# venkovic/julia-phd-krylov-spdes

Hardware: AMD Instinct MI355X
Metric: Schur-PCG iterations/sec (NN-preconditioned, assembled local Schurs), 1M DoF (higher is better)
Workload: dtype f64; 1 GPU; configs[2]: N=1000 structured P1 mesh, 996004 free DoF, 8 subdomains (4x2 boxes), lognormal a=exp(g) seed 481456, n_Γ=3989; pcg(S, b_schur, 0, ΠSnn), eps=1e-07; subdomains_per_gpu=8, parallelism=single GPU, it=15

## Files before the change

### julia-phd-krylov-spdes_amd/csrc/kernels.hpp

```cpp
#pragma once
#include <hip/hip_runtime.h>

#include "exchange_dev.hpp"
#include "spmv_blocks.hpp"

namespace mi {

constexpr int NT = 256;
constexpr int MAX_PARTS = 512;

struct SolverState {
  double rTr, rTz;
  double rTr_prev, rTz_prev;
  double d, alpha, beta;
  double tol, bnorm, eps;
  long long it, maxit, res_cap;
  long long it_nxt;
  int done;
  int overflow;
  int x0_zero;
};

struct PinnedFlags {
  long long it;
  int done;
  int overflow;
  int respec;
  int x0z;
  long long t_entry, t_exit;
  unsigned long long seq;
};
struct SolveArgs {
  const double *b_in, *x_in;
  double *x_out, *res_stage;
  double eps;
  long long maxit, res_cap, ncap;
  unsigned long long seq;
};

__device__ __forceinline__ double wave_sum(double v) {
#pragma unroll
  for (int off = 32; off > 0; off >>= 1) v += __shfl_down(v, off, 64);
  return v;
}
template <int NTH>
__device__ __forceinline__ double block_sum_t(double v, double *sm) {
  constexpr int NW = NTH / 64;
  v = wave_sum(v);
  const int lane = threadIdx.x & 63, w = threadIdx.x >> 6;
  if (lane == 0) sm[w] = v;
  __syncthreads();
  double t = lane < NW ? sm[lane] : 0.0;
#pragma unroll
  for (int off = NW / 2; off > 0; off >>= 1) t += __shfl_down(t, off, 64);
  t = __shfl(t, 0, 64);
  __syncthreads();
  return t;
}
__device__ __forceinline__ double block_sum(double v, double *sm) { return block_sum_t<NT>(v, sm); }
template <int NTH>
__device__ __forceinline__ void block_sum2_t(double &a, double &b, double *sm) {
// ... 941 lines not shown
  double *res_norm;
  const int *tgt;
  const int *peer;
  const int *jrank;
  int W;
  const unsigned long long *in_epoch;
  long long in_stride;
  const XchgPeers *xp;
  XchgState *xst;
  long long out_stride;
  unsigned int n_arrive;
  const XchgPeers *xpw;
  int x_inwait;
  int nvec;
  long long n_gamma;
  const double *AW;
  double *part_mu;
  const double *wm_loc;
  const SolveArgs *exit_args;
  PinnedFlags *exit_flags;
  long long *dbg;
  int dbg_wg;
};
#define MI_FSTAMP(i) \
  do { if (f.dbg && (int)blockIdx.x == f.dbg_wg && threadIdx.x == 0) f.dbg[dbg_row * 8 + (i)] = wall_clock64(); } while (0)
__device__ __forceinline__ double slot_sum(const double *slots, int g, int W) {
  double s = 0.0;
  if (W == 4) {
    const double4 q = *reinterpret_cast<const double4 *>(slots + 4ll * g);
    s += q.x; s += q.y; s += q.z; s += q.w;
  } else if (W == 2) {
    const double2 q = *reinterpret_cast<const double2 *>(slots + 2ll * g);
    s += q.x; s += q.y;
  } else {
    for (int j = 0; j < W; ++j) s += slots[(long long)g * W + j];
  }
  return s;
}

template <int RPW, int PHASE, int FOLD_CPT, int WAVES, bool XCHG, typename MT = double>
__global__ __launch_bounds__(64 * WAVES) void k_gemv_pcg(DenseMeta m, PcgFold f) {
  constexpr int NTH = 64 * WAVES, NR = WAVES * RPW;
  SolverState *st = f.st;
  const bool x_push = XCHG && f.xp != nullptr, x_inwait = XCHG && f.x_inwait != 0;
  const GemvTile t = m.tiles[blockIdx.x];
  const int done0 = st->done;
  const long long it0 = st->it, it_nxt0 = st->it_nxt, maxit = st->maxit, cap = st->res_cap;
  const double tol = st->tol, rTz0 = st->rTz, old = st->rTz_prev;
  const unsigned long long xo = XCHG && f.xst ? (x_inwait ? f.xst->xep[PHASE] : f.xst->epoch) : 0ull;
  const unsigned long long xe = x_inwait ? xo : (f.in_epoch ? *f.in_epoch : 0ull);
  asm volatile("" ::"s"(t.mat_off), "s"(t.n), "s"(t.ld), "s"(t.loc_off), "s"(t.row0), "s"(t.active), "s"(t.nrows), "s"(it0),
               "s"(it_nxt0), "s"(maxit), "s"(cap), "s"(tol), "s"(rTz0), "s"(old), "s"(done0), "s"(xe), "s"(xo));
  if (done0) return;
  GemvRows<RPW, MT> rows;
  if (x_inwait && f.in_stride) {
    if (t.active) rows.begin(m, t);
    if (threadIdx.x < 64) xchg_wait(f.xst, *f.xpw, xo);
    __syncthreads();
    if (__hip_atomic_load(&f.xst->err, __ATOMIC_RELAXED, __HIP_MEMORY_SCOPE_AGENT)) return;
  }
  const bool streaming = x_inwait && f.in_stride;
  const long long xoff = (long long)(xe & 1ull) * f.in_stride;
  const double *con_in = f.con_in + xoff, *part_in0 = f.part_in0 + xoff, *part_in1 = PHASE == 0 ? f.part_in1 + xoff : nullptr;
  __shared__ __attribute__((aligned(16))) double xs[GEMV_PANEL];
  __shared__ double sm[2 * (NTH / 64)];
  __shared__ double rowv[NR], rowc0[NR], rowc1[NR];
  __shared__ double rowy[NR];
  __shared__ int rowg[NR];
  const int off = t.loc_off, W = f.W, n = t.n;
  const bool lead = blockIdx.x == 0 && threadIdx.x == 0;
  if (threadIdx.x < NR) { rowc0[threadIdx.x] = 0.0; rowv[threadIdx.x] = 0.0; rowy[threadIdx.x] = 0.0; rowg[threadIdx.x] = 0; }
#if !MI355_OPERAND_FIRST
  if (t.active && !streaming) rows.begin(m, t);
#endif

  const bool first1 = PHASE == 1 && it_nxt0 == 0;
  const int dbg_row = (int)((PHASE == 1 ? 2 * it_nxt0 : 2 * it0 + 1) & 63);
  MI_FSTAMP(0);
  double pa = 0.0, pb = 0.0;
  for (int i0 = threadIdx.x; i0 < f.n_in; i0 += 8 * NTH) {
    double ta[8], tb[8];
#pragma unroll
    for (int k = 0; k < 8; ++k) {
      const int i = i0 + k * NTH;
      ta[k] = i < f.n_in ? part_in0[i] : 0.0;
      tb[k] = PHASE == 0 && i < f.n_in ? part_in1[i] : 0.0;
    }
#pragma unroll
    for (int k = 0; k < 8; ++k) { pa += ta[k]; if (PHASE == 0) pb += tb[k]; }
  }
  double cv[FOLD_CPT], cs[FOLD_CPT], cc[FOLD_CPT];
#pragma unroll
  for (int q = 0; q < FOLD_CPT; ++q) {
    const int j = q * NTH + threadIdx.x;
    cv[q] = cs[q] = 0.0; cc[q] = PHASE == 1 ? 1.0 : 0.0;
    if (j < n) {
      const int loc = off + j;
      cs[q] = slot_sum(con_in, loc, W);
      if (PHASE == 1) { cv[q] = first1 ? f.r_gamma[m.gidx[loc]] : f.r_cur[loc]; cc[q] = m.cnt[loc]; }
      else { cv[q] = f.p_cur[loc]; if (f.nvec > 0) cc[q] = f.wm_loc[loc]; }
    }
  }
  int o_q = -1, o_g = 0;
  bool o_own = false;
  double o_a = 0.0, o_x = 0.0;
  int o_peer[4] = {-1, -1, -1, -1};
#pragma unroll
  for (int q = 0; q < FOLD_CPT; ++q) {
    const int j = q * NTH + threadIdx.x, ri = j - t.row0;
    if (j < n && ri >= 0 && ri < t.nrows) {
      const int loc = off + j;
      o_q = q;
      o_own = f.jrank[loc] == 0;
      if (PHASE == 1) { o_a = first1 ? 0.0 : f.p_nxt[loc]; o_g = m.gidx[loc]; }
      else o_a = f.r_nxt[loc];
#pragma unroll
      for (int k = 0; k < 4; ++k) if (k < W) o_peer[k] = f.peer[loc * W + k];
    }
  }
  if (PHASE == 1 && o_q >= 0 && o_own) o_x = f.x[o_g];
  int e_tgt[RPW][4];
  double e_cnt[RPW];
#pragma unroll
  for (int k = 0; k < RPW; ++k) {
    const int r = t.row0 + (int)(threadIdx.x >> 6) * RPW + k;
    e_cnt[k] = 1.0;
#pragma unroll
    for (int q = 0; q < 4; ++q) e_tgt[k][q] = -1;
    if ((threadIdx.x & 63) == 0 && r < n) {
      const int loc = off + r;
      if (PHASE == 1) e_cnt[k] = m.cnt[loc];
#pragma unroll
      for (int q = 0; q < 4; ++q) if (q < W) e_tgt[k][q] = f.tgt[loc * W + q];
    }
  }

  int x_tgt = -1;
  if (x_push && t.active && threadIdx.x < 4 * NR) {
    const int r = t.row0 + (int)(threadIdx.x >> 2), k = threadIdx.x & 3;
    if (r < n && k < W) x_tgt = f.tgt[(off + r) * W + k];
  }
#if MI355_OPERAND_FIRST
  if (t.active && !streaming) rows.begin(m, t);
#endif
  MI_FSTAMP(1);
  double coef;
  if (PHASE == 1) {
    const bool first = first1;
    block_sum2_t<NTH>(pa, pb, sm);
    const double d = pa;
    coef = first ? 0.0 : rTz0 / d;
    if (lead) {
      st->d = d; st->alpha = coef;
      st->rTz_prev = first ? 1.0 : rTz0;
      st->it = it_nxt0;
      if (x_inwait) { f.xst->xep[0] = xo + (x_push ? 1 : 0); f.xst->epoch = xo; }
    }
  } else {
    const long long it_new = it0 + 1;
    block_sum2_t<NTH>(pa, pb, sm);
    const double rr = pa, rz = pb;
    const double res = sqrt(rr);
    const bool stop = !((it_new < maxit) && (res > tol));
    coef = 1. / old;
    coef *= rz;
    if (lead) {
      st->rTr = rr; st->rTz = rz; st->beta = coef;
      st->it_nxt = it_new;
      if (it_new <= cap) f.res_norm[it_new - 1] = res; else st->overflow = 1;
      if (stop || it_new > cap) st->done = 1;
      if (x_inwait) { f.xst->xep[1] = xo + (x_push && !(stop || it_new > cap) ? 1 : 0); f.xst->epoch = xo; }
    }
    if (stop || it_new > cap) {
      if (f.exit_args && blockIdx.x == 0) {
        const SolveArgs q = *f.exit_args;
        for (long long i = threadIdx.x; i < f.n_gamma; i += NTH) q.x_out[i] = f.x[i];
        if (q.res_stage) {
          const long long mres = it_new < q.ncap ? it_new : q.ncap;
          for (long long i = threadIdx.x; i < mres; i += NTH) q.res_stage[i] = i == it_new - 1 ? res : f.res_norm[i];
        }
        __threadfence_system();
        __syncthreads();
        if (threadIdx.x == 0) {
          PinnedFlags *fl = f.exit_flags;
          fl->it = it_new; fl->done = 1; fl->overflow = it_new > cap; fl->respec = 0; fl->x0z = st->x0_zero;
          fl->t_exit = wall_clock64();
          __threadfence_system();
          __hip_atomic_store(&fl->seq, q.seq, __ATOMIC_RELEASE, __HIP_MEMORY_SCOPE_SYSTEM);
        }
      }
      return;
    }
  }

  MI_FSTAMP(2);
#pragma unroll
  for (int q = 0; q < FOLD_CPT; ++q) {
    const int j = q * NTH + threadIdx.x;
    if (j < t.ld) {
      double v = 0.0, vs = 0.0;
      if (j < n) {
        v = PHASE == 1 ? (first1 ? cv[q] : cv[q] + (-coef) * cs[q])
                       : coef * cv[q] + cs[q];
        if (PHASE == 0 && f.nvec > 0) v = v - cc[q];
        vs = PHASE == 1 ? v / cc[q] : v;
      }
      xs[j] = vs;
      if (q == o_q) {
        const int ri = j - t.row0;
// ... 87 lines not shown
        const XchgPeers &P = *f.xp;
        const char *own = P.arena[P.rank];
        for (int q = 0; q < P.n; ++q) {
          const long long d = P.arena[q] - own;
          xchg_store(reinterpret_cast<double *>(reinterpret_cast<char *>(f.part_out0) + d) + xpo + ps, PHASE == 1 ? b : a);
          if (PHASE == 1) xchg_store(reinterpret_cast<double *>(reinterpret_cast<char *>(f.part_out1) + d) + xpo + ps, a);
        }
      }
    }
  }
  if (x_push) {
    asm volatile("s_waitcnt vmcnt(0)" ::: "memory");
    __syncthreads();
    if (threadIdx.x == 0) {
      const unsigned int prev = __hip_atomic_fetch_add(&f.xst->arrived, 1u, __ATOMIC_RELAXED, __HIP_MEMORY_SCOPE_AGENT);
      if (prev == f.n_arrive - 1) {
        __hip_atomic_store(&f.xst->arrived, 0u, __ATOMIC_RELAXED, __HIP_MEMORY_SCOPE_AGENT);
        const XchgPeers &P = *f.xp;
        for (int q = 0; q < P.n; ++q) __hip_atomic_store(xchg_flag(P, q, P.rank), xo + 1, __ATOMIC_RELAXED, __HIP_MEMORY_SCOPE_SYSTEM);
      }
    }
  }
  MI_FSTAMP(6);
}

__global__ __launch_bounds__(NT) void k_assemble(int n, const int *__restrict__ aptr, const int *__restrict__ apos,
                                                 const double *__restrict__ yloc, double *__restrict__ y,
                                                 const int *done) {
  if (done && *done) return;
  for (int i = blockIdx.x * NT + threadIdx.x; i < n; i += gridDim.x * NT) {
    double s = 0.0;
    for (int k = aptr[i]; k < aptr[i + 1]; ++k) s += yloc[apos[k]];
    y[i] = s;
  }
}
__global__ __launch_bounds__(NT) void k_assemble_slots(int n, int width, const double *__restrict__ yslots,
                                                       double *__restrict__ y, const int *done) {
  if (done && *done) return;
  for (int i = blockIdx.x * NT + threadIdx.x; i < n; i += gridDim.x * NT) {
    double s = 0.0;
    for (int j = 0; j < width; ++j) s += yslots[(long long)i * width + j];
    y[i] = s;
  }
}
__global__ __launch_bounds__(NT) void k_gather(int nloc, const int *__restrict__ gidx, const double *__restrict__ x,
                                               double *__restrict__ xcat) {
// ... 151 lines not shown
  }
  if (blockIdx.x == 0 && threadIdx.x == 0) {
    st->rTr = rr; st->rTz = rz; st->beta = beta;
    const long long it = st->it + 1;
    st->it = it;
    const double res = sqrt(rr);
    const bool over = it > st->res_cap;
    if (!over) res_norm[it - 1] = res; else st->overflow = 1;
    st->done = over || !((it < st->maxit) && (res > st->tol));
  }
}
__global__ __launch_bounds__(NT) void k_solve_begin(int n, const double *__restrict__ b_in, const double *__restrict__ x_in,
                                                    double *__restrict__ b, double *__restrict__ x, SolverState *st, double eps,
                                                    long long maxit, long long res_cap) {
  int nz = 0;
  for (int i = blockIdx.x * NT + threadIdx.x; i < n; i += gridDim.x * NT) {
    const double xi = x_in[i];
    b[i] = b_in[i]; x[i] = xi;
    nz |= xi != 0.0;
  }
  if (__syncthreads_or(nz) && threadIdx.x == 0) st->x0_zero = 0;
  if (blockIdx.x == 0 && threadIdx.x == 0) { st->eps = eps; st->maxit = maxit; st->res_cap = res_cap; st->done = 0; }
}
__device__ __forceinline__ unsigned long long sys_load_u64(const void *p) {
  return __hip_atomic_load((const unsigned long long *)p, __ATOMIC_RELAXED, __HIP_MEMORY_SCOPE_SYSTEM);
}
__global__ __launch_bounds__(NT) void k_solve_begin_g(int n, const SolveArgs *pin, double *__restrict__ b, double *__restrict__ x,
                                                      SolverState *st, SolveArgs *dev, PinnedFlags *flags) {
  __shared__ unsigned long long a[sizeof(SolveArgs) / 8];
  if (blockIdx.x == 0 && threadIdx.x == 0) flags->t_entry = wall_clock64();
  static_assert(sizeof(SolveArgs) % 8 == 0 && sizeof(SolveArgs) / 8 <= 64, "SolveArgs is a block of 8-byte fields");
  if (threadIdx.x < sizeof(SolveArgs) / 8) a[threadIdx.x] = sys_load_u64((const unsigned long long *)pin + threadIdx.x);
  __syncthreads();
  const SolveArgs &q = *reinterpret_cast<const SolveArgs *>(a);
  const double *b_in = q.b_in, *x_in = q.x_in;
  int nz = 0;
  for (int i = blockIdx.x * NT + threadIdx.x; i < n; i += gridDim.x * NT) {
    const double xi = x_in[i];
    b[i] = b_in[i]; x[i] = xi;
    nz |= xi != 0.0;
  }
  if (__syncthreads_or(nz) && threadIdx.x == 0) st->x0_zero = 0;
  if (blockIdx.x == 0) {
    if (threadIdx.x < sizeof(SolveArgs) / 8) ((unsigned long long *)dev)[threadIdx.x] = a[threadIdx.x];
    if (threadIdx.x == 0) { st->eps = q.eps; st->maxit = q.maxit; st->res_cap = q.res_cap; st->done = 0; }
  }
}
__global__ __launch_bounds__(NT) void k_solve_end_g(int n, SolverState *st, const SolveArgs *dev, int fold, const double *__restrict__ x,
                                                    const double *__restrict__ res_norm, PinnedFlags *flags, int *x0_zero,
                                                    unsigned *end_count) {
  __shared__ int last;
  const long long it = fold ? st->it_nxt : st->it;
  const SolveArgs q = *dev;
  if (sys_load_u64(&flags->seq) == q.seq) {
    if (blockIdx.x == 0 && threadIdx.x == 0) *x0_zero = 1;
    return;
  }
  for (int i = blockIdx.x * NT + threadIdx.x; i < n; i += gridDim.x * NT) q.x_out[i] = x[i];
  if (q.res_stage) {
    const long long m = it < q.ncap ? it : q.ncap;
    for (long long i = blockIdx.x * (long long)NT + threadIdx.x; i < m; i += (long long)gridDim.x * NT) q.res_stage[i] = res_norm[i];
  }
  __threadfence_system();
  __syncthreads();
  if (threadIdx.x == 0) last = atomicAdd(end_count, 1u) == gridDim.x - 1;
  __syncthreads();
  if (last && threadIdx.x == 0) {
    *end_count = 0;
    flags->it = it; flags->done = st->done; flags->overflow = st->overflow; flags->respec = 0; flags->x0z = *x0_zero;
    flags->t_exit = wall_clock64();
    *x0_zero = 1;
    __threadfence_system();
    __hip_atomic_store(&flags->seq, q.seq, __ATOMIC_RELEASE, __HIP_MEMORY_SCOPE_SYSTEM);
  }
}
__global__ __launch_bounds__(NT) void k_solve_end(int n, const SolverState *st, int fold, const double *__restrict__ x,
                                                  double *__restrict__ x_out, const double *__restrict__ res_norm,
// ... 376 lines not shown
__global__ __launch_bounds__(NTF) void k_entry_zero(int n, const SolveArgs *pin, double *__restrict__ b, double *__restrict__ x,
                                                    double *__restrict__ r, SolverState *st, SolveArgs *dev, PinnedFlags *flags) {
  __shared__ unsigned long long a[sizeof(SolveArgs) / 8];
  __shared__ double sm[NTF / 64 + 1];
  if (threadIdx.x == 0) flags->t_entry = wall_clock64();
  if (threadIdx.x < sizeof(SolveArgs) / 8) a[threadIdx.x] = sys_load_u64((const unsigned long long *)pin + threadIdx.x);
  __syncthreads();
  const SolveArgs &q = *reinterpret_cast<const SolveArgs *>(a);
  const double *b_in = q.b_in, *x_in = q.x_in;
  double bv[EPT], xv[EPT];
  int nz = 0;
#pragma unroll
  for (int k = 0; k < EPT; ++k) {
    const int e = k * NTF + threadIdx.x;
    bv[k] = 0.0; xv[k] = 0.0;
    if (e < n) { bv[k] = b_in[e]; xv[k] = x_in[e]; nz |= xv[k] != 0.0; }
  }
  nz = __syncthreads_or(nz);
  if (threadIdx.x < sizeof(SolveArgs) / 8) ((unsigned long long *)dev)[threadIdx.x] = a[threadIdx.x];
  if (nz) {
    if (threadIdx.x == 0) {
      st->done = 1; st->x0_zero = 0;
      flags->it = 0; flags->done = 0; flags->overflow = 0; flags->respec = 1; flags->x0z = 0;
      __threadfence_system();
      __hip_atomic_store(&flags->seq, q.seq, __ATOMIC_RELEASE, __HIP_MEMORY_SCOPE_SYSTEM);
    }
    return;
  }
  double srr = 0.0, sbb = 0.0;
#pragma unroll
  for (int k = 0; k < EPT; ++k) {
    const int e = k * NTF + threadIdx.x;
    if (e < n) {
      const double bi = bv[k];
      const double ri = bi - 0.0;
      b[e] = bi; x[e] = xv[k]; r[e] = ri;
      srr += ri * ri;
      sbb += bi * bi;
    }
  }
  srr = block_sum_f(srr, sm);
  sbb = block_sum_f(sbb, sm);
  if (threadIdx.x == 0) {
    st->eps = q.eps; st->maxit = q.maxit; st->res_cap = q.res_cap; st->x0_zero = 1;
    st->rTr = srr; st->bnorm = sqrt(sbb);
    st->tol = q.eps * st->bnorm;
// ... 140 lines not shown
```

### julia-phd-krylov-spdes_amd/csrc/operators.hpp

```cpp
#pragma once
#include <algorithm>
#include <atomic>
#include <cfloat>
#include <cmath>
#include <cstdlib>
#include <functional>
#include <numeric>

#include "common.hpp"
#include "kernels.hpp"
#include "assembly.hpp"
#include "exchange.hpp"

namespace mi {

inline int vec_grid(int64_t n) {
  int64_t g = (n + (int64_t)NT * 4 - 1) / ((int64_t)NT * 4);
  return (int)std::max<int64_t>(1, std::min<int64_t>(g, MAX_PARTS));
}
inline int env_int(const char *name, int dflt) {
  const char *s = std::getenv(name);
  return s && *s ? std::atoi(s) : dflt;
}
inline int to_i32(int64_t v, int64_t lo, int64_t hi, const char *what) {
// ... 461 lines not shown
    hipLaunchKernelGGL(k_assemble_slots, dim3(vec_grid(n)), dim3(NT), 0, ctx->stream, (int)n, maps.slot_width,
                       reduce_over_ranks ? yslots_all.p : yslots.p, y, done);
    MI_HIP(hipGetLastError());
  }
  DenseBlockOp *as_dense() override { return this; }
  void set_blocks(const double *src);
  static constexpr int KV = 4;
  DevBuf<double> yslots_multi;
  void apply_multi(const double *X, int64_t ldx, int k, double *Y, int64_t ldy) override {
    if (reduce_over_ranks || !ntiles || f32() || env_int("MI355_NO_MULTI", 0)) { Operator::apply_multi(X, ldx, k, Y, ldy); return; }
    const long long stride = (long long)n * maps.slot_width + 4;
    if (yslots_multi.n < (size_t)(stride * KV)) { yslots_multi.alloc((size_t)(stride * KV)); yslots_multi.zero(ctx->stream); }
    for (int v0 = 0; v0 < k; v0 += KV) {
      const int kv = std::min(KV, k - v0);
      const double *Xv = X + (size_t)v0 * ldx;
#define MI_GM(S) hipLaunchKernelGGL((k_gemv_multi<2, KV, S, 16>), dim3(ntiles), dim3(1024), 0, ctx->stream, meta, Xv, (long long)ldx, kv, yslots_multi.p, stride)
      if (scale) MI_GM(true); else MI_GM(false);
#undef MI_GM
      hipLaunchKernelGGL(k_assemble_slots_multi, dim3(vec_grid(n), kv), dim3(NT), 0, ctx->stream, (int)n, maps.slot_width,
                         yslots_multi.p, stride, Y + (size_t)v0 * ldy, (long long)ldy);
    }
    MI_HIP(hipGetLastError());
  }
  void gemv_pcg(int phase, const PcgFold &f) {
    if (!ntiles) return;
    ++folded_pcg_launches();
    const bool xchg = f.xp != nullptr || f.x_inwait != 0;
    if (f32() && (phase != 1 || xchg)) raise(MI_ERR_BAD_ARG, "folded PCG launch: no fp32 kernel for phase %d%s", phase, xchg ? " with peer exchange" : "");
#define MI_PCG4(R, P, C, V) do { if (xchg) hipLaunchKernelGGL((k_gemv_pcg<R, P, C, V, true>), dim3(ntiles), dim3(64 * V), 0, ctx->stream, meta, f); \
                                 else hipLaunchKernelGGL((k_gemv_pcg<R, P, C, V, false>), dim3(ntiles), dim3(64 * V), 0, ctx->stream, meta, f); } while (0)
#define MI_PCG32(R, C, V) hipLaunchKernelGGL((k_gemv_pcg<R, 1, C, V, false, float>), dim3(ntiles), dim3(64 * V), 0, ctx->stream, meta, f)
#define MI_PCG3(R, C, V) do { if (f32()) MI_PCG32(R, C, V); else if (phase) MI_PCG4(R, 1, C, V); else MI_PCG4(R, 0, C, V); } while (0)
#define MI_PCG2(R, V) do { const int c = (max_ld + 64 * V - 1) / (64 * V); \
                           if (c <= 2) MI_PCG3(R, 2, V); else if (c == 3) MI_PCG3(R, 3, V); else if (c == 4) MI_PCG3(R, 4, V); \
                           else if (c == 5) MI_PCG3(R, 5, V); else if (c == 6) MI_PCG3(R, 6, V); else MI_PCG3(R, 8, V); } while (0)
#define MI_PCG(R) do { if (waves == 16) MI_PCG2(R, 16); else if (waves == 8) MI_PCG2(R, 8); else MI_PCG2(R, 4); } while (0)
    if (rpw == 1) MI_PCG(1); else if (rpw == 2) MI_PCG(2); else MI_PCG(4);
#undef MI_PCG
#undef MI_PCG2
#undef MI_PCG3
#undef MI_PCG32
#undef MI_PCG4
    MI_HIP(hipGetLastError());
  }
  bool same_maps(const DenseBlockOp &o) const {
    return n == o.n && maps.slot_width == o.maps.slot_width && maps.nd == o.maps.nd && maps.gidx_h == o.maps.gidx_h;
  }
  AsmView view_of(double *) override {
    return reduce_over_ranks ? AsmView{yslots_all.p, maps.slot_width} : AsmView{yslots.p, maps.slot_width};
  }
  AsmView apply_view(const double *x, double *y, const int *done) override {
    gemv(x, done);
    if (!reduce_over_ranks) return AsmView{yslots.p, maps.slot_width};
    ctx->allreduce(yslots.p, yslots_all.p, (size_t)n * maps.slot_width);
    return AsmView{yslots_all.p, maps.slot_width};
  }
  void bytes(int64_t *a, int64_t *d) const override { *a = alg_bytes + 8 * n; *d = alg_bytes; }
  void apply_dominant(const double *x) override { gemv(x, nullptr); }
};

template <typename MT>
__global__ __launch_bounds__(NT) void k_block_to_rowmajor(int n, int ld, const double *__restrict__ src, MT *__restrict__ dstm) {
// ... 490 lines not shown
```

### julia-phd-krylov-spdes_amd/csrc/solvers.hpp

```cpp
#pragma once
#include <atomic>
#include <chrono>
#include <cmath>
#include <cstddef>
#include <tuple>

#include "eig_kernels.hpp"
#include "operators.hpp"
#ifdef MI355_EXPERIMENTAL
#include "resident.hpp"
#endif

namespace mi {


constexpr int64_t RES_STAGE = 8192;
constexpr int CF_VEC_GRID = 256;

struct GraphKey {
  const Operator *A, *M;
  int nvec, chunk;
  int tag = 0;
  bool operator<(const GraphKey &o) const {
    return std::tie(A, M, nvec, chunk, tag) < std::tie(o.A, o.M, o.nvec, o.chunk, o.tag);
// ... 126 lines not shown
  double *res_stage = nullptr;
  hipEvent_t ev[2] = {nullptr, nullptr};
  std::map<GraphKey, hipGraphExec_t> graphs;
  std::map<GraphKey, int> predicted;
  std::map<GraphKey, bool> zero_x0;
  std::map<std::pair<const Operator *, const Operator *>, std::unique_ptr<ResidentPlan>> resident;

  explicit SolverWorkspace(int64_t n_) : n(n_), g(vec_grid(n_)) {
    auto pad = [](size_t b) { return (b + 255) / 256 * 256; };
    const size_t vec = pad(sizeof(double) * ((size_t)n + 2)), part = pad(sizeof(double) * MAX_PARTS);
    const size_t total = pad(sizeof(SolverState)) + 4 * part + 6 * vec;
    slab.alloc(total);
    memset_sync(slab.p, 0, total);
    char *q = slab.p;
    st = (SolverState *)q; q += pad(sizeof(SolverState));
    part_pAp = (double *)q; q += part; part_rr = (double *)q; q += part;
    part_rz = (double *)q; q += part; part_bb = (double *)q; q += part;
    r = (double *)q; q += vec; z = (double *)q; q += vec; p = (double *)q; q += vec;
    Ap = (double *)q; q += vec; x = (double *)q; q += vec; b = (double *)q; q += vec;
    MI_HIP(hipHostMalloc((void **)&flags, 2 * sizeof(PinnedFlags)));
    std::memset(flags, 0, 2 * sizeof(PinnedFlags));
    MI_HIP(hipHostMalloc((void **)&args, sizeof(SolveArgs)));
    if (env_int("MI355_FOLD_DEBUG", 0)) { fold_dbg.alloc(512); memset_sync(fold_dbg.p, 0, 512 * sizeof(long long)); }
    args_dev.alloc(1); end_count.alloc(1);
    memset_sync(end_count.p, 0, sizeof(unsigned));
    MI_HIP(hipHostMalloc((void **)&res_stage, RES_STAGE * sizeof(double)));
    for (auto &e : ev) MI_HIP(hipEventCreateWithFlags(&e, hipEventDisableTiming));
  }
  ~SolverWorkspace() {
    drop_graphs();
    if (flags) (void)hipHostFree(flags);
    if (args) (void)hipHostFree(args);
    if (res_stage) (void)hipHostFree(res_stage);
    for (auto &e : ev) if (e) (void)hipEventDestroy(e);
  }
  void drop_graphs() {
    for (auto &kv : graphs) (void)hipGraphExecDestroy(kv.second);
    graphs.clear();
  }
  void drop_graphs_of(const Operator *op) {
    for (auto it = graphs.begin(); it != graphs.end();)
      if (it->first.A == op || it->first.M == op) { (void)hipGraphExecDestroy(it->second); it = graphs.erase(it); }
      else ++it;
    for (auto it = predicted.begin(); it != predicted.end();)
      if (it->first.A == op || it->first.M == op) it = predicted.erase(it);
      else ++it;
    for (auto it = zero_x0.begin(); it != zero_x0.end();)
// ... 45 lines not shown
    const double piv_inv = 1.0 / a[k + (size_t)k * n];
    for (int i = k + 1; i < n; ++i) a[i + (size_t)k * n] *= piv_inv;
    for (int j = k + 1; j < n; ++j) {
      const double akj = a[k + (size_t)j * n];
      for (int i = k + 1; i < n; ++i) a[i + (size_t)j * n] -= a[i + (size_t)k * n] * akj;
    }
  }
  return 0;
}

struct Krylov {
  mi_ctx_s *ctx;
  Operator *A, *M;
  SolverWorkspace &ws;
  int nvec;
  int n, g;
  hipStream_t s;
  bool fused;
  bool fold;
  CsrDev *Ac = nullptr;
  bool csrfold() const { return Ac != nullptr && !eig.tag; }
  DenseBlockOp *Ad = nullptr, *Md = nullptr;
  int capture_whole = 0;
  struct EigHook {
    int tag = 0, spdim = 0;
    bool has_tvec = false;
    bool project_r = false;
  } eig;
  std::vector<double> gram_host;

  Krylov(mi_ctx_s *c, Operator *A_, Operator *M_, int nvec_, bool generic = false, bool allow_fold = true)
      : ctx(c), A(A_), M(M_), ws(workspace(c, A_->n)), nvec(nvec_), n((int)A_->n), g(ws.g), s(c->stream),
        fused(!generic && A_->n <= FUSED_MAX_N && !env_int("MI355_NO_FUSED", 0)), fold(false) {
    const bool big_fold = !fused && !generic && nvec_ == 0 && !env_int("MI355_NO_FUSED", 0) && !env_int("MI355_NO_BIG_FOLD", 0);
    if ((fused || big_fold) && allow_fold && M && nvec <= 64 && !env_int("MI355_NO_FOLD", 0) && !(nvec > 0 && env_int("MI355_NO_FOLD_DEFL", 0))) {
      Ad = A->as_dense(); Md = M->as_dense();
      fold = Ad && Md && (!Ad->reduce_over_ranks || (Ad->full_maps && nvec == 0)) &&
             (!Md->reduce_over_ranks || (Md->full_maps && Md->fold_p1_off && nvec == 0 && !env_int("MI355_NO_FOLD_SHARDED_NN", 0))) &&
             !Ad->scale && Md->scale && Ad->same_maps(*Md) && Ad->ntiles > 0 && Ad->max_ld <= GEMV_PANEL && Md->max_ld <= GEMV_PANEL &&
             Ad->maps.slot_width <= 4 &&
             !(Md->f32() && Md->reduce_over_ranks) &&
             (Ad->max_ld + 64 * Ad->waves - 1) / (64 * Ad->waves) <= 8 && (Md->max_ld + 64 * Md->waves - 1) / (64 * Md->waves) <= 8;
    }
    const double *dv = nullptr;
    if (!fused && nvec == 0 && A->as_csr() && A->as_csr()->nblocks > 0 && (!M || M->diag_kind(&dv) != 0) && !env_int("MI355_NO_CSRFOLD", 0))
      Ac = A->as_csr();
// ... 57 lines not shown
    return fused && nvec == 0 ? M->view_of(ws.z) : AsmView{ws.z, 0};
  }
  AsmView Ap_view() const { return fused ? A->view_of(ws.Ap) : AsmView{ws.Ap, 0}; }
  void eig_record() {
    const int pre = M != nullptr;
    double *tv = eig.has_tvec ? ws.etvec.p : nullptr;
    hipLaunchKernelGGL(k_eig_vec, dim3(g), dim3(NT), 0, s, n, ws.st, ws.ees.p, pre, eig.spdim, z_view(), Ap_view(), ws.eV.p, tv);
    if (eig.has_tvec)
      hipLaunchKernelGGL(k_eig_coupling, dim3(g, 2 * ws.e_nvec), dim3(NT), 0, s, n, ws.st, ws.ees.p, ws.eV.p, ws.etvec.p,
                         ws.epart.p);
    hipLaunchKernelGGL(k_eig_state, dim3(1), dim3(64), 0, s, ws.st, ws.ees.p, ws.eT.p, eig.spdim, ws.epart.p, g,
                       (int)eig.has_tvec);
    MI_HIP(hipGetLastError());
  }

#define MI_EPT_DISPATCH(CALL)            \
  do {                                   \
    if (n <= NTF) { CALL(1); }           \
    else if (n <= 2 * NTF) { CALL(2); }  \
    else if (n <= 4 * NTF) { CALL(4); }  \
    else { CALL(8); }                    \
  } while (0)

  void iteration() {
    const int *dn = done();
    const int pre = M != nullptr;
    const double *Wp = nvec > 0 ? ws.W.p : nullptr, *mup = nvec > 0 ? ws.mu.p : nullptr;
    if (fold) {
      Md->gemv_pcg(1, fold_args(1));
      if (Md->reduce_over_ranks) Md->reduce_fold(dn, inwait());
      if (nvec > 0) {
        hipLaunchKernelGGL(k_defl_mu, dim3((Ad->maps.nloc + 1023) / 1024), dim3(1024), 0, s, ws.st, nvec, Md->ntiles, ws.fold_mu.p,
                           ws.LU.p, ws.piv.p, ws.W.p, (long long)n, Ad->maps.nloc, Ad->maps.gidx.p, ws.fold_wm.p, ws.mu.p, ws.fold_wloc.p);
        MI_HIP(hipGetLastError());
      }
      Ad->gemv_pcg(0, fold_args(0));
      if (Ad->reduce_over_ranks) Ad->reduce_fold(dn, inwait());
      return;
    }
    if (fused) {
      const AsmView vAp = A->apply_view(ws.p, ws.Ap, dn);
      if (!pre && nvec == 0) {
#define MI_CALL(E) hipLaunchKernelGGL((k_fused_cg<E>), dim3(1), dim3(NTF), 0, s, n, ws.st, vAp, ws.p, ws.x, ws.r, ws.res_norm.p)
        MI_EPT_DISPATCH(MI_CALL);
#undef MI_CALL
        if (eig.tag) eig_record();
        MI_HIP(hipGetLastError());
        return;
      }
#define MI_CALL(E) hipLaunchKernelGGL((k_fused_xr<E>), dim3(1), dim3(NTF), 0, s, n, ws.st, vAp, ws.p, ws.x, ws.r, pre)
      MI_EPT_DISPATCH(MI_CALL);
#undef MI_CALL
// ... 111 lines not shown
        dot_partial(ws.r, ws.z, ws.part_rz, nullptr);
      }
      hipLaunchKernelGGL(k_csrfold_start, dim3(g), dim3(NT), 0, s, n, CF_VEC_GRID, ws.st, ws.part_rr, ws.part_bb,
                         diag == 2 ? ws.part_rz : (const double *)nullptr, g, diag == 2 ? ws.z : ws.r, ws.cf_pz.p, ws.cf_rr.p,
                         ws.cf_rz.p);
      MI_HIP(hipGetLastError());
      return;
    }
    const double *zz = ws.r;
    if (pre) {
      M->apply(ws.r, ws.z, nullptr);
      dot_partial(ws.r, ws.z, ws.part_rz, nullptr);
      zz = ws.z;
    }
    hipLaunchKernelGGL(k_init_state, dim3(1), dim3(NT), 0, s, ws.st, ws.part_rr, ws.part_bb,
                       pre ? ws.part_rz : (const double *)nullptr, g, ws.res_norm.p);
    if (nvec > 0) project(ws.AW.p, zz, nullptr);
    hipLaunchKernelGGL(k_init_p, dim3(g), dim3(NT), 0, s, n, zz, ws.p, nvec > 0 ? ws.W.p : (const double *)nullptr,
                       nvec > 0 ? ws.mu.p : (const double *)nullptr, nvec);
    MI_HIP(hipGetLastError());
  }

  hipGraphExec_t graph(int chunk, int whole = 0) {
    GraphKey key{A, M, nvec, chunk, eig.tag * 8 + (fused ? 1 : 0) + (fold ? 2 : 0) + (csrfold() ? 4 : 0) + 1024 * whole};
    auto it = ws.graphs.find(key);
    if (it != ws.graphs.end()) return it->second;
    hipGraph_t gr = nullptr;
    MI_HIP(hipStreamBeginCapture(s, hipStreamCaptureModeThreadLocal));
    try {
      capture_whole = whole;
      if (whole == 2) {
#define MI_CALL(E) hipLaunchKernelGGL((k_entry_zero<E>), dim3(1), dim3(NTF), 0, s, n, ws.args, ws.b, ws.x, ws.r, ws.st, ws.args_dev.p, &ws.flags[0])
        MI_EPT_DISPATCH(MI_CALL);
#undef MI_CALL
        MI_HIP(hipGetLastError());
      } else {
        if (whole) {
          hipLaunchKernelGGL(k_solve_begin_g, dim3(g), dim3(NT), 0, s, n, ws.args, ws.b, ws.x, ws.st, ws.args_dev.p, &ws.flags[0]);
          MI_HIP(hipGetLastError());
        }
        if (chunk < 0) setup_tail();
      }
      for (int k = 0; k < std::abs(chunk); ++k) iteration();
      capture_whole = 0;
      if (whole) {
        hipLaunchKernelGGL(k_solve_end_g, dim3(g), dim3(NT), 0, s, n, ws.st, ws.args_dev.p, (int)(fold || csrfold()), ws.x, ws.res_norm.p,
                           &ws.flags[0], &ws.st->x0_zero, ws.end_count.p);
        MI_HIP(hipGetLastError());
      }
    } catch (...) {
      capture_whole = 0;
      (void)hipStreamEndCapture(s, &gr);
      if (gr) (void)hipGraphDestroy(gr);
      throw;
    }
    MI_HIP(hipStreamEndCapture(s, &gr));
    hipGraphExec_t ex = nullptr;
    hipError_t e = hipGraphInstantiate(&ex, gr, nullptr, nullptr, 0);
    (void)hipGraphDestroy(gr);
    if (e != hipSuccess) raise(MI_ERR_HIP, "hipGraphInstantiate failed: %s", hipGetErrorString(e));
    ws.graphs[key] = ex;
    return ex;
  }

  void wait_seq(unsigned long long seq) {
    volatile unsigned long long *f = &ws.flags[0].seq;
// ... 120 lines not shown
        for (int k = 0; k < 512 && h[k]; ++k) std::fprintf(stderr, "%s%.2f", (k >= 5 && (k - 5) % 8 == 0) ? "\n  " : " ", (h[k] - h[0]) * 0.01);
        std::fprintf(stderr, "\n");
      }
      if (ws.flags[0].done) {
        rp->epoch += (unsigned long long)(2 * ws.flags[0].it + 4);
        ran_resident = true;
        use_graph = false;
      } else {
        rp->reset(s);
        rp->usable = false;
        int64_t mx = maxit, cd = 0; double e = eps;
        begin(b_in, x_io, W_in, mx, e, cd);
      }
    }
#endif
    if (use_graph) {
      const GraphKey pk{A, M, nvec, 0};
      int &predicted = ws.predicted[pk];
      int64_t first = predicted > 0 ? predicted : ctx->chunk;
      if (first > 64) first -= first % 32;
      first = std::max<int64_t>(1, std::min<int64_t>(first, std::min<int64_t>(maxit, 1024)));
      if (ws.graphs.size() > 48) ws.drop_graphs();
      bool zero_variant = whole && fold && fused && ws.zero_x0[pk] && !env_int("MI355_NO_ZERO_ENTRY", 0);
      hipGraphExec_t g0 = nullptr;
      try {
        g0 = graph(-(int)first, whole ? (zero_variant ? 2 : 1) : 0);
      } catch (const Error &) {
        if (!ctx->comm) throw;
        ctx->no_graph = true;
        use_graph = false;
      }
      if (use_graph) {
      if (whole) {
        const unsigned long long seq = ++ws.seq;
        *ws.args = SolveArgs{b_in, x_io, x_io, spec_res ? ws.res_stage : (double *)nullptr, eps, (long long)maxit, (long long)cap_dev,
                             (long long)ncap, seq};
        ++ctx->n_replays; MI_HIP(hipGraphLaunch(g0, s));
        wait_seq(seq);
        if (ws.flags[0].respec) {
          zero_variant = false;
          ws.zero_x0[pk] = false;
          g0 = graph(-(int)first, 1);
          const unsigned long long seq2 = ++ws.seq;
          ws.args->seq = seq2;
          ++ctx->n_replays; MI_HIP(hipGraphLaunch(g0, s));
          wait_seq(seq2);
        }
        if (fold) ws.zero_x0[pk] = ws.flags[0].x0z != 0;
        if (ws.stats_on) ws.stat(ws.flags[0].t_exit - ws.flags[0].t_entry);
        if (ws.fold_dbg.p && fold) {
          std::vector<long long> h(512);
          MI_HIP(hipStreamSynchronize(s));
          memcpy_sync(h.data(), ws.fold_dbg.p, 512 * sizeof(long long), hipMemcpyDeviceToHost);
          const long long t0 = h[0] ? h[0] : ws.flags[0].t_entry;
          std::fprintf(stderr, "[fold stamps] wg %d, entry kernel at %.2f us\n", env_int("MI355_FOLD_DEBUG_WG", 0), (ws.flags[0].t_entry - t0) * 0.01);
          for (int r = 0; r < 64 && h[r * 8]; ++r) {
            std::fprintf(stderr, "  launch %2d:", r);
            for (int k = 0; k < 7; ++k) std::fprintf(stderr, " %8.2f", h[r * 8 + k] ? (h[r * 8 + k] - t0) * 0.01 : -1.0);
            std::fprintf(stderr, "\n");
// ... 60 lines not shown
```

Before: 32210 iterations/s.

## Fold the zero-guess solve entry into the first preconditioner launch

Folds the separate single-block k_entry_zero kernel (reads pinned args, checks x0==0, sets r=b, norms, state init) into the first ΠS folded PCG launch via an ENTRY template variant. It also introduces a slim kernel-argument struct with compile-time nulls for unused fields, and replaces a system-scope pinned-memory read in the end kernel with a device-side seq copy. The aim is to remove one serialized kernel launch and a host-memory load from each solve. In exchange, block 0 of the first launch does extra entry work, and the kernel gains more template variants and complexity.

New measurement: 30480 iterations/s. 5.4% lower.

```diff
diff --git a/julia-phd-krylov-spdes_amd/csrc/kernels.hpp b/julia-phd-krylov-spdes_amd/csrc/kernels.hpp
--- a/julia-phd-krylov-spdes_amd/csrc/kernels.hpp
+++ b/julia-phd-krylov-spdes_amd/csrc/kernels.hpp
@@ -37,6 +37,10 @@
   long long maxit, res_cap, ncap;
   unsigned long long seq;
 };
+
+__device__ __forceinline__ unsigned long long sys_load_u64(const void *p) {
+  return __hip_atomic_load((const unsigned long long *)p, __ATOMIC_RELAXED, __HIP_MEMORY_SCOPE_SYSTEM);
+}
 
 __device__ __forceinline__ double wave_sum(double v) {
 #pragma unroll
@@ -1024,6 +1028,51 @@
   long long *dbg;
   int dbg_wg;
 };
+struct PcgFoldSlim {
+  SolverState *st;
+  const double *con_in;
+  double *con_out;
+  const double *part_in0, *part_in1;
+  double *part_out0, *part_out1;
+  double *r_cur, *r_nxt, *p_cur, *p_nxt;
+  double *x;
+  const double *r_gamma;
+  double *res_norm;
+  const int *tgt, *peer, *jrank;
+  const SolveArgs *exit_args;
+  PinnedFlags *exit_flags;
+  long long n_gamma;
+  int n_in, W;
+  static constexpr const unsigned long long *in_epoch = nullptr;
+  static constexpr long long in_stride = 0, out_stride = 0;
+  static constexpr const XchgPeers *xp = nullptr, *xpw = nullptr;
+  static constexpr XchgState *xst = nullptr;
+  static constexpr unsigned int n_arrive = 0;
+  static constexpr int x_inwait = 0, nvec = 0, dbg_wg = 0;
+  static constexpr const double *AW = nullptr, *wm_loc = nullptr;
+  static constexpr double *part_mu = nullptr;
+  static constexpr long long *dbg = nullptr;
+  PcgFoldSlim() = default;
+  explicit PcgFoldSlim(const PcgFold &f)
+      : st(f.st), con_in(f.con_in), con_out(f.con_out), part_in0(f.part_in0), part_in1(f.part_in1), part_out0(f.part_out0),
+        part_out1(f.part_out1), r_cur(f.r_cur), r_nxt(f.r_nxt), p_cur(f.p_cur), p_nxt(f.p_nxt), x(f.x), r_gamma(f.r_gamma),
+        res_norm(f.res_norm), tgt(f.tgt), peer(f.peer), jrank(f.jrank), exit_args(f.exit_args), exit_flags(f.exit_flags),
+        n_gamma(f.n_gamma), n_in(f.n_in), W(f.W) {}
+  static bool fits(const PcgFold &f) {
+    return !f.in_epoch && !f.in_stride && !f.xp && !f.xst && !f.xpw && !f.x_inwait && f.nvec == 0 && !f.dbg;
+  }
+};
+struct PcgEntry {
+  const SolveArgs *pin;
+  double *b;
+  SolveArgs *dev;
+  PinnedFlags *flags;
+};
+struct PcgFoldEntry : PcgFoldSlim {
+  PcgEntry en;
+  PcgFoldEntry() = default;
+  PcgFoldEntry(const PcgFold &f, const PcgEntry &e) : PcgFoldSlim(f), en(e) {}
+};
 #define MI_FSTAMP(i) \
   do { if (f.dbg && (int)blockIdx.x == f.dbg_wg && threadIdx.x == 0) f.dbg[dbg_row * 8 + (i)] = wall_clock64(); } while (0)
 __device__ __forceinline__ double slot_sum(const double *slots, int g, int W) {
@@ -1040,19 +1089,28 @@
   return s;
 }
 
-template <int RPW, int PHASE, int FOLD_CPT, int WAVES, bool XCHG, typename MT = double>
-__global__ __launch_bounds__(64 * WAVES) void k_gemv_pcg(DenseMeta m, PcgFold f) {
+template <int RPW, int PHASE, int FOLD_CPT, int WAVES, bool XCHG, typename MT = double, typename FA = PcgFold, bool ENTRY = false>
+__global__ __launch_bounds__(64 * WAVES) void k_gemv_pcg(DenseMeta m, FA f) {
   constexpr int NTH = 64 * WAVES, NR = WAVES * RPW;
+  static_assert(!ENTRY || (PHASE == 1 && !XCHG && NTH == 1024), "the ENTRY launch is a ΠS launch of 1024 threads (the sum tree of k_entry_zero)");
+  constexpr int NARG = sizeof(SolveArgs) / 8;
+  static_assert(sizeof(SolveArgs) % 8 == 0 && NARG <= 64, "SolveArgs is a block of 8-byte fields");
   SolverState *st = f.st;
   const bool x_push = XCHG && f.xp != nullptr, x_inwait = XCHG && f.x_inwait != 0;
+  __shared__ unsigned long long ea[ENTRY ? NARG : 1];
+  if constexpr (ENTRY) {
+    if (blockIdx.x == 0 && threadIdx.x == 0) f.en.flags->t_entry = wall_clock64();
+    if ((int)threadIdx.x < (blockIdx.x == 0 ? NARG : 2)) ea[threadIdx.x] = sys_load_u64((const unsigned long long *)f.en.pin + threadIdx.x);
+  }
   const GemvTile t = m.tiles[blockIdx.x];
-  const int done0 = st->done;
-  const long long it0 = st->it, it_nxt0 = st->it_nxt, maxit = st->maxit, cap = st->res_cap;
-  const double tol = st->tol, rTz0 = st->rTz, old = st->rTz_prev;
+  const int done0 = ENTRY ? 0 : st->done;
+  const long long it0 = ENTRY ? 0 : st->it, it_nxt0 = ENTRY ? 0 : st->it_nxt, maxit = ENTRY ? 0 : st->maxit, cap = ENTRY ? 0 : st->res_cap;
+  const double tol = ENTRY ? 0.0 : st->tol, rTz0 = ENTRY ? 0.0 : st->rTz, old = ENTRY ? 1.0 : st->rTz_prev;
   const unsigned long long xo = XCHG && f.xst ? (x_inwait ? f.xst->xep[PHASE] : f.xst->epoch) : 0ull;
   const unsigned long long xe = x_inwait ? xo : (f.in_epoch ? *f.in_epoch : 0ull);
-  asm volatile("" ::"s"(t.mat_off), "s"(t.n), "s"(t.ld), "s"(t.loc_off), "s"(t.row0), "s"(t.active), "s"(t.nrows), "s"(it0),
-               "s"(it_nxt0), "s"(maxit), "s"(cap), "s"(tol), "s"(rTz0), "s"(old), "s"(done0), "s"(xe), "s"(xo));
+  if constexpr (!ENTRY)
+    asm volatile("" ::"s"(t.mat_off), "s"(t.n), "s"(t.ld), "s"(t.loc_off), "s"(t.row0), "s"(t.active), "s"(t.nrows), "s"(it0),
+                 "s"(it_nxt0), "s"(maxit), "s"(cap), "s"(tol), "s"(rTz0), "s"(old), "s"(done0), "s"(xe), "s"(xo));
   if (done0) return;
   GemvRows<RPW, MT> rows;
   if (x_inwait && f.in_stride) {
@@ -1076,7 +1134,7 @@
   if (t.active && !streaming) rows.begin(m, t);
 #endif
 
-  const bool first1 = PHASE == 1 && it_nxt0 == 0;
+  const bool first1 = ENTRY || (PHASE == 1 && it_nxt0 == 0);
   const int dbg_row = (int)((PHASE == 1 ? 2 * it_nxt0 : 2 * it0 + 1) & 63);
   MI_FSTAMP(0);
   double pa = 0.0, pb = 0.0;
@@ -1092,14 +1150,17 @@
     for (int k = 0; k < 8; ++k) { pa += ta[k]; if (PHASE == 0) pb += tb[k]; }
   }
   double cv[FOLD_CPT], cs[FOLD_CPT], cc[FOLD_CPT];
+  [[maybe_unused]] int cg[ENTRY ? FOLD_CPT : 1];
 #pragma unroll
   for (int q = 0; q < FOLD_CPT; ++q) {
     const int j = q * NTH + threadIdx.x;
     cv[q] = cs[q] = 0.0; cc[q] = PHASE == 1 ? 1.0 : 0.0;
+    if constexpr (ENTRY) cg[q] = 0;
     if (j < n) {
       const int loc = off + j;
-      cs[q] = slot_sum(con_in, loc, W);
-      if (PHASE == 1) { cv[q] = first1 ? f.r_gamma[m.gidx[loc]] : f.r_cur[loc]; cc[q] = m.cnt[loc]; }
+      if constexpr (!ENTRY) cs[q] = slot_sum(con_in, loc, W);
+      if constexpr (ENTRY) { cg[q] = m.gidx[loc]; cc[q] = m.cnt[loc]; }
+      else if (PHASE == 1) { cv[q] = first1 ? f.r_gamma[m.gidx[loc]] : f.r_cur[loc]; cc[q] = m.cnt[loc]; }
       else { cv[q] = f.p_cur[loc]; if (f.nvec > 0) cc[q] = f.wm_loc[loc]; }
     }
   }
@@ -1120,7 +1181,7 @@
       for (int k = 0; k < 4; ++k) if (k < W) o_peer[k] = f.peer[loc * W + k];
     }
   }
-  if (PHASE == 1 && o_q >= 0 && o_own) o_x = f.x[o_g];
+  if (PHASE == 1 && !ENTRY && o_q >= 0 && o_own) o_x = f.x[o_g];
   int e_tgt[RPW][4];
   double e_cnt[RPW];
 #pragma unroll
@@ -1141,6 +1202,15 @@
   if (x_push && t.active && threadIdx.x < 4 * NR) {
     const int r = t.row0 + (int)(threadIdx.x >> 2), k = threadIdx.x & 3;
     if (r < n && k < W) x_tgt = f.tgt[(off + r) * W + k];
+  }
+  if constexpr (ENTRY) {
+    __syncthreads();
+    const double *b_in = reinterpret_cast<const double *>(ea[0]), *x_in = reinterpret_cast<const double *>(ea[1]);
+#pragma unroll
+    for (int q = 0; q < FOLD_CPT; ++q)
+      if (q * NTH + (int)threadIdx.x < n) cv[q] = b_in[cg[q]];
+    if (o_q >= 0 && o_own) o_x = x_in[o_g];
+    if (blockIdx.x == 0 && threadIdx.x < NARG) reinterpret_cast<unsigned long long *>(f.en.dev)[threadIdx.x] = ea[threadIdx.x];
   }
 #if MI355_OPERAND_FIRST
   if (t.active && !streaming) rows.begin(m, t);
@@ -1187,6 +1257,7 @@
           PinnedFlags *fl = f.exit_flags;
           fl->it = it_new; fl->done = 1; fl->overflow = it_new > cap; fl->respec = 0; fl->x0z = st->x0_zero;
           fl->t_exit = wall_clock64();
+          const_cast<SolveArgs *>(f.exit_args)[1].seq = q.seq;
           __threadfence_system();
           __hip_atomic_store(&fl->seq, q.seq, __ATOMIC_RELEASE, __HIP_MEMORY_SCOPE_SYSTEM);
         }
@@ -1320,6 +1391,54 @@
     }
   }
   MI_FSTAMP(6);
+  if constexpr (ENTRY) {
+    if (blockIdx.x != 0) return;
+    const SolveArgs &q = *reinterpret_cast<const SolveArgs *>(ea);
+    const double *b_in = q.b_in, *x_in = q.x_in;
+    const int ng = (int)f.n_gamma;
+    double bv[8];
+    int nz = 0;
+#pragma unroll
+    for (int k = 0; k < 8; ++k) {
+      const int e = k * NTH + threadIdx.x;
+      bv[k] = 0.0;
+      if (e < ng) { bv[k] = b_in[e]; nz |= x_in[e] != 0.0; }
+    }
+    nz = __syncthreads_or(nz);
+    if (nz) {
+      if (threadIdx.x == 0) {
+        PinnedFlags *fl = f.en.flags;
+        st->done = 1; st->x0_zero = 0;
+        fl->it = 0; fl->done = 0; fl->overflow = 0; fl->respec = 1; fl->x0z = 0;
+        f.en.dev[1].seq = q.seq;
+        __threadfence_system();
+        __hip_atomic_store(&fl->seq, q.seq, __ATOMIC_RELEASE, __HIP_MEMORY_SCOPE_SYSTEM);
+      }
+      return;
+    }
+    double srr = 0.0, sbb = 0.0;
+#pragma unroll
+    for (int k = 0; k < 8; ++k) {
+      const int e = k * NTH + threadIdx.x;
+      if (e < ng) {
+        const double bi = bv[k];
+        const double ri = bi - 0.0;
+        f.en.b[e] = bi; const_cast<double *>(f.r_gamma)[e] = ri;
+        srr += ri * ri;
+        sbb += bi * bi;
+      }
+    }
+    srr = block_sum_t<NTH>(srr, sm);
+    sbb = block_sum_t<NTH>(sbb, sm);
+    if (threadIdx.x == 0) {
+      st->eps = q.eps; st->maxit = q.maxit; st->res_cap = q.res_cap; st->x0_zero = 1;
+      st->rTr = srr; st->bnorm = sqrt(sbb);
+      st->tol = q.eps * st->bnorm;
+      st->it = 0; st->it_nxt = 0; st->done = 0; st->overflow = 0;
+      st->rTz = 0.0; st->rTz_prev = 1.0; st->rTr_prev = srr;
+      st->alpha = 0.0; st->beta = 0.0;
+    }
+  }
 }
 
 __global__ __launch_bounds__(NT) void k_assemble(int n, const int *__restrict__ aptr, const int *__restrict__ apos,
@@ -1517,9 +1636,6 @@
   if (__syncthreads_or(nz) && threadIdx.x == 0) st->x0_zero = 0;
   if (blockIdx.x == 0 && threadIdx.x == 0) { st->eps = eps; st->maxit = maxit; st->res_cap = res_cap; st->done = 0; }
 }
-__device__ __forceinline__ unsigned long long sys_load_u64(const void *p) {
-  return __hip_atomic_load((const unsigned long long *)p, __ATOMIC_RELAXED, __HIP_MEMORY_SCOPE_SYSTEM);
-}
 __global__ __launch_bounds__(NT) void k_solve_begin_g(int n, const SolveArgs *pin, double *__restrict__ b, double *__restrict__ x,
                                                       SolverState *st, SolveArgs *dev, PinnedFlags *flags) {
   __shared__ unsigned long long a[sizeof(SolveArgs) / 8];
@@ -1547,7 +1663,7 @@
   __shared__ int last;
   const long long it = fold ? st->it_nxt : st->it;
   const SolveArgs q = *dev;
-  if (sys_load_u64(&flags->seq) == q.seq) {
+  if (dev[1].seq == q.seq) {
     if (blockIdx.x == 0 && threadIdx.x == 0) *x0_zero = 1;
     return;
   }
@@ -1970,6 +2086,7 @@
     if (threadIdx.x == 0) {
       st->done = 1; st->x0_zero = 0;
       flags->it = 0; flags->done = 0; flags->overflow = 0; flags->respec = 1; flags->x0z = 0;
+      dev[1].seq = q.seq;
       __threadfence_system();
       __hip_atomic_store(&flags->seq, q.seq, __ATOMIC_RELEASE, __HIP_MEMORY_SCOPE_SYSTEM);
     }
diff --git a/julia-phd-krylov-spdes_amd/csrc/operators.hpp b/julia-phd-krylov-spdes_amd/csrc/operators.hpp
--- a/julia-phd-krylov-spdes_amd/csrc/operators.hpp
+++ b/julia-phd-krylov-spdes_amd/csrc/operators.hpp
@@ -507,22 +507,36 @@
     }
     MI_HIP(hipGetLastError());
   }
-  void gemv_pcg(int phase, const PcgFold &f) {
+  bool entry_capable() const { return waves == 16 && !reduce_over_ranks; }
+  void gemv_pcg(int phase, const PcgFold &f, const PcgEntry *entry = nullptr) {
     if (!ntiles) return;
     ++folded_pcg_launches();
     const bool xchg = f.xp != nullptr || f.x_inwait != 0;
     if (f32() && (phase != 1 || xchg)) raise(MI_ERR_BAD_ARG, "folded PCG launch: no fp32 kernel for phase %d%s", phase, xchg ? " with peer exchange" : "");
+    const bool slim = !xchg && PcgFoldSlim::fits(f) && !env_int("MI355_FAT_ARGS", 0);
+    if (entry && (phase != 1 || !slim || !entry_capable())) raise(MI_ERR_BAD_ARG, "folded PCG launch: no entry form for this launch");
+    const PcgFoldSlim fs = slim ? PcgFoldSlim(f) : PcgFoldSlim();
+    const PcgFoldEntry fe = entry ? PcgFoldEntry(f, *entry) : PcgFoldEntry();
 #define MI_PCG4(R, P, C, V) do { if (xchg) hipLaunchKernelGGL((k_gemv_pcg<R, P, C, V, true>), dim3(ntiles), dim3(64 * V), 0, ctx->stream, meta, f); \
+                                 else if (slim) hipLaunchKernelGGL((k_gemv_pcg<R, P, C, V, false, double, PcgFoldSlim>), dim3(ntiles), dim3(64 * V), 0, ctx->stream, meta, fs); \
                                  else hipLaunchKernelGGL((k_gemv_pcg<R, P, C, V, false>), dim3(ntiles), dim3(64 * V), 0, ctx->stream, meta, f); } while (0)
-#define MI_PCG32(R, C, V) hipLaunchKernelGGL((k_gemv_pcg<R, 1, C, V, false, float>), dim3(ntiles), dim3(64 * V), 0, ctx->stream, meta, f)
+#define MI_PCG32(R, C, V) do { if (slim) hipLaunchKernelGGL((k_gemv_pcg<R, 1, C, V, false, float, PcgFoldSlim>), dim3(ntiles), dim3(64 * V), 0, ctx->stream, meta, fs); \
+                               else hipLaunchKernelGGL((k_gemv_pcg<R, 1, C, V, false, float>), dim3(ntiles), dim3(64 * V), 0, ctx->stream, meta, f); } while (0)
 #define MI_PCG3(R, C, V) do { if (f32()) MI_PCG32(R, C, V); else if (phase) MI_PCG4(R, 1, C, V); else MI_PCG4(R, 0, C, V); } while (0)
+#define MI_PCGE(R, C) do { if (f32()) hipLaunchKernelGGL((k_gemv_pcg<R, 1, C, 16, false, float, PcgFoldEntry, true>), dim3(ntiles), dim3(1024), 0, ctx->stream, meta, fe); \
+                           else hipLaunchKernelGGL((k_gemv_pcg<R, 1, C, 16, false, double, PcgFoldEntry, true>), dim3(ntiles), dim3(1024), 0, ctx->stream, meta, fe); } while (0)
 #define MI_PCG2(R, V) do { const int c = (max_ld + 64 * V - 1) / (64 * V); \
                            if (c <= 2) MI_PCG3(R, 2, V); else if (c == 3) MI_PCG3(R, 3, V); else if (c == 4) MI_PCG3(R, 4, V); \
                            else if (c == 5) MI_PCG3(R, 5, V); else if (c == 6) MI_PCG3(R, 6, V); else MI_PCG3(R, 8, V); } while (0)
-#define MI_PCG(R) do { if (waves == 16) MI_PCG2(R, 16); else if (waves == 8) MI_PCG2(R, 8); else MI_PCG2(R, 4); } while (0)
+#define MI_PCG2E(R) do { const int c = (max_ld + 1023) / 1024; \
+                         if (c <= 2) MI_PCGE(R, 2); else if (c == 3) MI_PCGE(R, 3); else if (c == 4) MI_PCGE(R, 4); \
+                         else if (c == 5) MI_PCGE(R, 5); else if (c == 6) MI_PCGE(R, 6); else MI_PCGE(R, 8); } while (0)
+#define MI_PCG(R) do { if (entry) MI_PCG2E(R); else if (waves == 16) MI_PCG2(R, 16); else if (waves == 8) MI_PCG2(R, 8); else MI_PCG2(R, 4); } while (0)
     if (rpw == 1) MI_PCG(1); else if (rpw == 2) MI_PCG(2); else MI_PCG(4);
 #undef MI_PCG
+#undef MI_PCG2E
 #undef MI_PCG2
+#undef MI_PCGE
 #undef MI_PCG3
 #undef MI_PCG32
 #undef MI_PCG4
diff --git a/julia-phd-krylov-spdes_amd/csrc/solvers.hpp b/julia-phd-krylov-spdes_amd/csrc/solvers.hpp
--- a/julia-phd-krylov-spdes_amd/csrc/solvers.hpp
+++ b/julia-phd-krylov-spdes_amd/csrc/solvers.hpp
@@ -172,7 +172,8 @@
     std::memset(flags, 0, 2 * sizeof(PinnedFlags));
     MI_HIP(hipHostMalloc((void **)&args, sizeof(SolveArgs)));
     if (env_int("MI355_FOLD_DEBUG", 0)) { fold_dbg.alloc(512); memset_sync(fold_dbg.p, 0, 512 * sizeof(long long)); }
-    args_dev.alloc(1); end_count.alloc(1);
+    args_dev.alloc(2); end_count.alloc(1);
+    memset_sync(args_dev.p, 0, 2 * sizeof(SolveArgs));
     memset_sync(end_count.p, 0, sizeof(unsigned));
     MI_HIP(hipHostMalloc((void **)&res_stage, RES_STAGE * sizeof(double)));
     for (auto &e : ev) MI_HIP(hipEventCreateWithFlags(&e, hipEventDisableTiming));
@@ -264,6 +265,15 @@
   bool csrfold() const { return Ac != nullptr && !eig.tag; }
   DenseBlockOp *Ad = nullptr, *Md = nullptr;
   int capture_whole = 0;
+  bool entry_folded() const {
+    return fold && fused && nvec == 0 && Md->entry_capable() && !ws.fold_dbg.p && !inwait() && !env_int("MI355_FAT_ARGS", 0) &&
+           !env_int("MI355_NO_ENTRY_FOLD", 0);
+  }
+  bool head_launch() const { return entry_folded() && env_int("MI355_HEAD_LAUNCH", 0) != 0; }
+  void entry_launch() {
+    const PcgEntry en{ws.args, ws.b, ws.args_dev.p, &ws.flags[0]};
+    Md->gemv_pcg(1, fold_args(1), &en);
+  }
   struct EigHook {
     int tag = 0, spdim = 0;
     bool has_tvec = false;
@@ -367,12 +377,13 @@
     else { CALL(8); }                    \
   } while (0)
 
-  void iteration() {
+  void iteration(int first = 0) {
     const int *dn = done();
     const int pre = M != nullptr;
     const double *Wp = nvec > 0 ? ws.W.p : nullptr, *mup = nvec > 0 ? ws.mu.p : nullptr;
     if (fold) {
-      Md->gemv_pcg(1, fold_args(1));
+      if (first == 1) entry_launch();
+      else if (first == 0) Md->gemv_pcg(1, fold_args(1));
       if (Md->reduce_over_ranks) Md->reduce_fold(dn, inwait());
       if (nvec > 0) {
         hipLaunchKernelGGL(k_defl_mu, dim3((Ad->maps.nloc + 1023) / 1024), dim3(1024), 0, s, ws.st, nvec, Md->ntiles, ws.fold_mu.p,
@@ -530,14 +541,18 @@
   }
 
   hipGraphExec_t graph(int chunk, int whole = 0) {
-    GraphKey key{A, M, nvec, chunk, eig.tag * 8 + (fused ? 1 : 0) + (fold ? 2 : 0) + (csrfold() ? 4 : 0) + 1024 * whole};
+    GraphKey key{A, M, nvec, chunk, eig.tag * 8 + (fused ? 1 : 0) + (fold ? 2 : 0) + (csrfold() ? 4 : 0) + 1024 * whole +
+                 (whole >= 2 && entry_folded() ? 8192 : 0)};
     auto it = ws.graphs.find(key);
     if (it != ws.graphs.end()) return it->second;
     hipGraph_t gr = nullptr;
     MI_HIP(hipStreamBeginCapture(s, hipStreamCaptureModeThreadLocal));
     try {
       capture_whole = whole;
-      if (whole == 2) {
+      const bool efold = whole >= 2 && entry_folded();
+      if (whole == 3 && !efold) raise(MI_ERR_BAD_ARG, "internal: head launch without the entry form");
+      if (efold) {
+      } else if (whole == 2) {
 #define MI_CALL(E) hipLaunchKernelGGL((k_entry_zero<E>), dim3(1), dim3(NTF), 0, s, n, ws.args, ws.b, ws.x, ws.r, ws.st, ws.args_dev.p, &ws.flags[0])
         MI_EPT_DISPATCH(MI_CALL);
 #undef MI_CALL
@@ -549,7 +564,7 @@
         }
         if (chunk < 0) setup_tail();
       }
-      for (int k = 0; k < std::abs(chunk); ++k) iteration();
+      for (int k = 0; k < std::abs(chunk); ++k) iteration(k == 0 && efold ? whole - 1 : 0);
       capture_whole = 0;
       if (whole) {
         hipLaunchKernelGGL(k_solve_end_g, dim3(g), dim3(NT), 0, s, n, ws.st, ws.args_dev.p, (int)(fold || csrfold()), ws.x, ws.res_norm.p,
@@ -716,9 +731,10 @@
       first = std::max<int64_t>(1, std::min<int64_t>(first, std::min<int64_t>(maxit, 1024)));
       if (ws.graphs.size() > 48) ws.drop_graphs();
       bool zero_variant = whole && fold && fused && ws.zero_x0[pk] && !env_int("MI355_NO_ZERO_ENTRY", 0);
+      const bool head = zero_variant && head_launch();
       hipGraphExec_t g0 = nullptr;
       try {
-        g0 = graph(-(int)first, whole ? (zero_variant ? 2 : 1) : 0);
+        g0 = graph(-(int)first, whole ? (zero_variant ? (head ? 3 : 2) : 1) : 0);
       } catch (const Error &) {
         if (!ctx->comm) throw;
         ctx->no_graph = true;
@@ -729,6 +745,7 @@
         const unsigned long long seq = ++ws.seq;
         *ws.args = SolveArgs{b_in, x_io, x_io, spec_res ? ws.res_stage : (double *)nullptr, eps, (long long)maxit, (long long)cap_dev,
                              (long long)ncap, seq};
+        if (head) entry_launch();
         ++ctx->n_replays; MI_HIP(hipGraphLaunch(g0, s));
         wait_seq(seq);
         if (ws.flags[0].respec) {
```
